# drdh/Homophily-MARL

Measured on AMD Instinct MI355X. Metric: agent_steps_per_sec, higher is better.
Workload: dtype fp32

## Files before the change

homophily_marl_amd/csrc/ssd_policy_mfma.hip:

```cpp
#include "ssd_policy_common.h"
#include <type_traits>

namespace ssd {
#define SSD_GLOBAL __attribute__((address_space(1)))

template <int V> using int_c = std::integral_constant<int, V>;
template <int... Vs, typename R, typename F>
static R pick(int v, R none, F&& f) {
    R r = none;
    ((v == Vs ? (void)(r = f(int_c<Vs>{})) : (void)0), ...);
    return r;
}

static int raise_lds_limit(const void* const* fns, int count, size_t bytes, bool (&done)[64]) {
    int dev = 0;
    if (hipGetDevice(&dev) != hipSuccess || dev < 0 || dev >= 64) return -1;
    if (done[dev]) return 0;
    for (int i = 0; i < count; ++i)
        if (hipFuncSetAttribute(fns[i], hipFuncAttributeMaxDynamicSharedMemorySize, (int)bytes) != hipSuccess) return -1;
    done[dev] = true;
    return 0;
}
static int raise_lds_limit(const void* fn, size_t bytes, bool (&done)[64]) { return raise_lds_limit(&fn, 1, bytes, done); }

// ... 227 lines not shown
    else if (C) asm volatile("s_load_dwordx16 %0, %2, %3\n\ts_load_dwordx4 %1, %2, %4\n\ts_waitcnt lgkmcnt(0)" : "=&s"(a), "=&s"(c) : "s"(ka), "s"(cold_base), "s"(cold_base + 128) : "memory");
    else asm volatile("s_load_dwordx16 %0, %1, %2\n\ts_waitcnt lgkmcnt(0)" : "=&s"(a) : "s"(ka), "s"(cold_base) : "memory");
    A = __builtin_bit_cast(ColdA, a);
    if (B) *B = __builtin_bit_cast(ColdB, b);
    if (C) *C = __builtin_bit_cast(ColdC, c);
#else
    (void)A; (void)B; (void)C;
#endif
}
#define COLD(T, field) cold_ptr<T>(COLD_BASE, (int)offsetof(HeadCold, field))
#define COLD_U64(field) ((uint64_t)cold_ptr<void>(COLD_BASE, (int)offsetof(HeadCold, field)))

template <int PREC>
struct Frag4 { u32x4 h[4], l[4]; };
template <int PREC>
__device__ __forceinline__ void frag4_load(const uint8_t* img, int c, int lane, Frag4<PREC>& f) {
#pragma unroll
    for (int ot = 0; ot < 4; ++ot) {
        const uint8_t* p = img + (size_t)step_piece<PREC>(c, 0, ot) * 1024 + lane * 16;
        f.h[ot] = *reinterpret_cast<const u32x4*>(p);
        if (PREC == 2) f.l[ot] = *reinterpret_cast<const u32x4*>(p + 4 * 1024);
    }
}
template <int PREC>
__device__ __forceinline__ void frag4_mma(const Frag4<PREC>& f, u32x4 bh, u32x4 bl, f32x4* acc) {
    if (PREC == 2) {
#pragma unroll
        for (int ot = 0; ot < 4; ++ot) acc[ot] = mma<PREC>(f.l[ot], bh, acc[ot]);
#pragma unroll
        for (int ot = 0; ot < 4; ++ot) acc[ot] = mma<PREC>(f.h[ot], bl, acc[ot]);
    }
#pragma unroll
    for (int ot = 0; ot < 4; ++ot) acc[ot] = mma<PREC>(f.h[ot], bh, acc[ot]);
}

template <int PREC>
__device__ __forceinline__ void operand(const f32x4 (&x)[4], float scale, u32x4 (&bh)[2], u32x4 (&bl)[2]) {
#pragma unroll
    for (int s = 0; s < 2; ++s) {
        float v[8];
#pragma unroll
        for (int j = 0; j < 8; ++j) v[j] = x[2 * s + (j >> 2)][j & 3] * scale;
        split8<PREC>(v, bh[s], bl[s]);
    }
}

__device__ __forceinline__ float amax2(float acc, float a, float b) {
#if defined(__HIP_DEVICE_COMPILE__)
    float r;
    asm("v_max3_f32 %0, |%1|, |%2|, %3" : "=v"(r) : "v"(a), "v"(b), "v"(acc));
    return r;
#else
    return fmaxf(acc, fmaxf(fabsf(a), fabsf(b)));
#endif
}
template <int NT>
__device__ __forceinline__ float amax_tiles(float acc, const f32x4 (&x)[NT]) {
#pragma unroll
    for (int t = 0; t < NT; ++t) { acc = amax2(acc, x[t][0], x[t][1]); acc = amax2(acc, x[t][2], x[t][3]); }
    return acc;
}

__device__ __forceinline__ float sigmoid_fast(float x) { return __builtin_amdgcn_rcpf(1.f + __expf(-x)); }
__device__ __forceinline__ float tanh_fast(float x) {
    const float ax = fminf(fabsf(x), 15.f);
    const float t = 1.f - 2.f * __builtin_amdgcn_rcpf(__expf(2.f * ax) + 1.f);
    return copysignf(t, x);
}

template <int INC>
struct TileIn {
    f32x4 x[4];
    f32x4 hp[4];
    int pa, act;
    int32_t inc[3];
    uint32_t rv;
    float pr, p0, p1, o0, o1;
    int aj[3];
    float f[3][7];
    float own[3], ep;
    int term;
};

template <typename T>
__device__ __forceinline__ T ld32(const T* base, uint32_t idx) {
    typedef const T SSD_GLOBAL gT;
    return *(gT*)((const uint8_t SSD_GLOBAL*)(const void SSD_GLOBAL*)base + (size_t)(idx * (uint32_t)sizeof(T)));
}
__device__ __forceinline__ void stg128(void* base, size_t byte_off, f32x4 v) {
    typedef f32x4 SSD_GLOBAL gv;
    *(gv*)((uint8_t SSD_GLOBAL*)(void SSD_GLOBAL*)base + byte_off) = v;
}
__device__ __forceinline__ f32x4 ldg128(const void* base, size_t byte_off) {
    typedef const f32x4 SSD_GLOBAL gv;
    return *(gv*)((const uint8_t SSD_GLOBAL*)(const void SSD_GLOBAL*)base + byte_off);
}
template <int INC, bool SMALL = false>
__device__ __forceinline__ void load_tile_rows(const HeadK& a, int tile, int agent, int lane, TileIn<INC>& in) {
    const int m = lane & 15, q = lane >> 4, N = a.N;
    const int b = tile * 16 + m, bc = b < N ? b : N - 1;
    const uint32_t arow = (uint32_t)agent * (uint32_t)N + (uint32_t)bc;
    const uint32_t ro = arow * 64u + 4u * (uint32_t)q;
#pragma unroll
    for (int ct = 0; ct < 4; ++ct) in.hp[ct] = ldg128(a.h, (size_t)((ro + 16u * ct) * 4u));
#pragma unroll
    for (int ct = 0; ct < (INC ? 4 : 2); ++ct) in.x[ct] = ldg128(a.inputs, (size_t)((ro + 16u * ct) * 4u));
    if constexpr (SMALL && !INC) {
        const uint32_t er = (uint32_t)bc * (uint32_t)a.n + (uint32_t)agent;
        in.pa = (int)ld32(reinterpret_cast<const int32_t*>(a.prev_actions), 2u * er);
        in.pr = ld32(a.prev_reward, er);
        in.rv = a.recv ? ld32(reinterpret_cast<const uint32_t*>(a.recv), arow * 4u + (uint32_t)q) : 0u;
        typedef float f32x2v __attribute__((ext_vector_type(2)));
        const f32x2v pp = ld32(reinterpret_cast<const f32x2v*>(a.pos), er);
        in.p0 = pp.x; in.p1 = pp.y;
    }
}
template <int INC, bool ROWS_DONE = false, bool SMALL_DONE = false>
__device__ __forceinline__ void load_tile(const HeadK& a, int tile, int agent, int lane, TileIn<INC>& in) {
    const int m = lane & 15, q = lane >> 4, N = a.N, n = a.n;
    const int b = tile * 16 + m, bc = b < N ? b : N - 1;
    const uint32_t arow = (uint32_t)agent * (uint32_t)N + (uint32_t)bc;
    const uint32_t ro = arow * 64u + 4u * (uint32_t)q;
    if (!ROWS_DONE) {
#pragma unroll
        for (int ct = 0; ct < 4; ++ct) in.hp[ct] = ldg128(a.h, (size_t)((ro + 16u * ct) * 4u));
    }
    if (!INC) {
        if (a.feat_part) {
            const uint32_t rows = (uint32_t)n * (uint32_t)N;
#pragma unroll
            for (int ct = 0; ct < 2; ++ct) {
                f32x4 part[6];
#pragma unroll
                for (int bd = 0; bd < 6; ++bd) {
                    const int bdc = bd < a.feat_bands ? bd : a.feat_bands - 1;
                    part[bd] = ldg128(a.feat_part, (size_t)((((uint32_t)bdc * rows + arow) * 32u + 16u * ct + 4u * q) * 4u));
                }
                f32x4 s = ldg128(a.lin_b, (size_t)((16 * ct + 4 * q) * 4));
#pragma unroll
                for (int bd = 0; bd < 6; ++bd) { const float on = bd < a.feat_bands ? 1.f : 0.f; s += part[bd] * on; }
                in.x[ct] = s;
            }
        } else if (!ROWS_DONE) {
            in.x[0] = ldg128(a.inputs, (size_t)(ro * 4u));
            in.x[1] = ldg128(a.inputs, (size_t)((ro + 16u) * 4u));
        }
        const uint32_t er = (uint32_t)bc * (uint32_t)n + (uint32_t)agent;
        if (!SMALL_DONE) {
            in.pa = (int)ld32(reinterpret_cast<const int32_t*>(a.prev_actions), 2u * er);
            in.pr = ld32(a.prev_reward, er);
        }
        if (a.recv) {
            if (!SMALL_DONE) in.rv = ld32(reinterpret_cast<const uint32_t*>(a.recv), arow * 4u + (uint32_t)q);
            in.inc[0] = in.inc[1] = in.inc[2] = 0;
        } else {
            in.rv = 0u;
            const int32_t* pi = reinterpret_cast<const int32_t*>(a.prev_inc);
#pragma unroll
            for (int k = 0; k < 3; ++k) {
                const int g = q + 4 * k;
                const uint32_t gc = (uint32_t)(g < n ? g : n - 1);
                in.inc[k] = (k == 0 || n > 4 * k) ? ld32(pi, 2u * (((uint32_t)bc * (uint32_t)n + gc) * (uint32_t)n + (uint32_t)agent)) : 0;
            }
        }
        typedef float f32x2v __attribute__((ext_vector_type(2)));
        if (!SMALL_DONE) {
            const f32x2v pp = ld32(reinterpret_cast<const f32x2v*>(a.pos), er);
            in.p0 = pp.x; in.p1 = pp.y;
        }
        const float* orient = a.orient ? a.orient : a.pos;
        const f32x2v oo = ld32(reinterpret_cast<const f32x2v*>(orient), er);
        in.o0 = oo.x; in.o1 = oo.y;
    } else {
        if (!ROWS_DONE) {
#pragma unroll
            for (int ct = 0; ct < 4; ++ct) in.x[ct] = ldg128(a.inputs, (size_t)((ro + 16u * ct) * 4u));
        }
        in.act = (int)ld32(reinterpret_cast<const int32_t*>(a.actions), 2u * ((uint32_t)bc * (uint32_t)n + (uint32_t)agent));
#pragma unroll
        for (int k = 0; k < 3; ++k) {
            const int it = lane + 64 * k, row = it / n, j = it - row * n, bb = tile * 16 + row;
            const bool live = it < 16 * n && bb < N;
            const uint32_t ej = live ? (uint32_t)bb * (uint32_t)n + (uint32_t)j : (uint32_t)N * (uint32_t)n - 1u;
            in.aj[k] = (int)ld32(reinterpret_cast<const int32_t*>(a.actions), 2u * ej);
            typedef float f32x2v __attribute__((ext_vector_type(2)));
            const f32x2v pj = ld32(reinterpret_cast<const f32x2v*>(a.pos_pre), ej), oj = ld32(reinterpret_cast<const f32x2v*>(a.orient_pre), ej);
            in.f[k][0] = pj.x; in.f[k][1] = pj.y; in.f[k][2] = oj.x; in.f[k][3] = oj.y;
            in.f[k][4] = ld32(a.reward, ej); in.f[k][5] = ld32(a.clean, ej); in.f[k][6] = ld32(a.den, ej);
        }
        {
            const int br = tile * 16 + (lane & 15), brc = br < N ? br : N - 1;
            const uint32_t ea = (uint32_t)brc * (uint32_t)n + (uint32_t)agent;
            in.own[0] = ld32(a.reward, ea); in.own[1] = ld32(a.clean, ea); in.own[2] = ld32(a.den, ea);
            in.ep = ld32(a.ep_ret ? a.ep_ret : a.reward, ea);
            in.term = (int)ld32(a.term ? a.term : reinterpret_cast<const uint8_t*>(a.reward), (uint32_t)brc);
        }
    }
}

__device__ __forceinline__ void refetch_head_args(HeadK& out, int k_off) {
#if defined(__HIP_DEVICE_COMPILE__)
    typedef __attribute__((address_space(4))) const uint32_t k_u32;
    uint64_t p = (uint64_t)(uintptr_t)__builtin_amdgcn_kernarg_segment_ptr();
    asm volatile("" : "+s"(p));
    k_u32* src = (k_u32*)(p + (uint64_t)k_off);
    uint32_t* dst = reinterpret_cast<uint32_t*>(&out);
#pragma unroll
    for (int i = 0; i < (int)(sizeof(HeadK) / 4); ++i) dst[i] = src[i];
#else
    (void)out;
#endif
}
static_assert(sizeof(HeadK) % 4 == 0, "HeadK is copied dword by dword");

template <int INC, int PREC, int AT, int GEN, int WAVES, bool LOOP = false, int KOFF = 0, bool PRE_SMALL = false>
__device__ __forceinline__ void head_body(const HeadK& a_entry, uint8_t* lds_raw, const int block) {
    constexpr int COLD_BASE = KOFF + HEAD_COLD_OFFSET;
    constexpr int IMAGE_BYTES = SSD_POLICY_IMAGE_BYTES(PREC);
    constexpr float XS = PREC == 2 ? HEAD_XSCALE : 1.f, INV = PREC == 2 ? 1.f / (HEAD_WSCALE * HEAD_XSCALE) : 1.f;
    const int tid = threadIdx.x, wave = __builtin_amdgcn_readfirstlane(tid >> 6);
    constexpr int A = AT;
    uint32_t seen = 0;
    bool first = true;
    volatile lds_u32* landed = (volatile lds_u32*)(lds_raw + IMAGE_BYTES + WAVES * SCRATCH * 4);
    TileIn<INC> in_rows;
    {
        const HeadK& a = a_entry;
        const int lane = tid & 63;
        (void)lane;
        PSTAMP(0);
        PSTAMP_REAL(14);
        if (!LOOP && wave < WAVES) {
            const int bia0 = block - (block / a.bpa) * a.bpa, tile00 = wave * a.bpa + bia0;
            if (tile00 < ((a.N + 15) >> 4)) load_tile_rows<INC, PRE_SMALL>(a, tile00, block / a.bpa, lane, in_rows);
        }
        if (!LOOP) {
            if (!INC) asm volatile("" :: "s"(a.N), "s"(a.n), "s"(a.bpa), "s"(a.h), "s"(a.inputs), "s"(a.weights), "s"(a.eps), "s"(a.step), "s"(a.t_index),
                                         "s"(a.prev_actions), "s"(a.prev_reward), "s"(a.recv), "s"(a.prev_inc), "s"(a.pos), "s"(a.orient), "s"(a.feat_part),
                                         "s"(a.lin_b), "s"(a.feat_bands), "s"(a.avail_bits), "s"(a.pos_scale));
            else asm volatile("" :: "s"(a.N), "s"(a.n), "s"(a.bpa), "s"(a.h), "s"(a.inputs), "s"(a.weights), "s"(a.eps), "s"(a.step), "s"(a.t_index),
                                    "s"(a.actions), "s"(a.pos_pre), "s"(a.orient_pre), "s"(a.reward), "s"(a.clean), "s"(a.den), "s"(a.ep_ret), "s"(a.term),
                                    "s"(a.inp), "s"(a.pos_scale));
        }
        if (wave == WAVES) *landed = 0u;
        __builtin_amdgcn_s_barrier();
        if (wave == WAVES) {
            const int agent = block / a.bpa;
            stream_image<PREC>(a.weights + (size_t)agent * IMAGE_BYTES + lane * 16, (uint32_t)(uintptr_t)lds_raw, landed);
            return;
        }
    }
    auto pass = [&](const HeadK& a, const int lane, const int tile) {
    const int agent = block / a.bpa;
    const int m = lane & 15, q = lane >> 4;
    const int N = a.N, n = a.n;
    const int tiles = (N + 15) >> 4;
    TileIn<INC> in;
    if constexpr (!LOOP) in = in_rows;
    if (!INC) PSTAMP_DRAINED(8);
    if (!INC) PSTAMP(9);
    float eps = *(const float SSD_GLOBAL*)a.eps;
    int64_t step64 = *(const int64_t SSD_GLOBAL*)a.step;
    long slot_t = a.t_index ? (long)*(const int64_t SSD_GLOBAL*)a.t_index : 0;
    if (tile < tiles) {
        if constexpr (LOOP) load_tile<INC, false>(a, tile, agent, lane, in);
// ... 258 lines not shown
            file_inputs(tile);
            hand_counters();
        }
        if (first) PSTAMP(4);
        u32x4 f2h[2], f2l[2];
#pragma unroll
        for (int s2 = 0; s2 < 2; ++s2) {
            const uint8_t* p2 = img + (size_t)fc2_piece<PREC>(0, s2) * 1024 + lane * 16;
            f2h[s2] = *reinterpret_cast<const u32x4*>(p2);
            if (PREC == 2) f2l[s2] = *reinterpret_cast<const u32x4*>(p2 + 2 * 1024);
        }
        f32x4 hn[4];
#pragma unroll
        for (int ft = 0; ft < 4; ++ft) {
            const f32x4 bir = *reinterpret_cast<const f32x4*>(tail + HT_BI + 16 * ft + 4 * q), bhr = *reinterpret_cast<const f32x4*>(tail + HT_BH + 16 * ft + 4 * q);
            const f32x4 biz = *reinterpret_cast<const f32x4*>(tail + HT_BI + 64 + 16 * ft + 4 * q), bhz = *reinterpret_cast<const f32x4*>(tail + HT_BH + 64 + 16 * ft + 4 * q);
            const f32x4 bin = *reinterpret_cast<const f32x4*>(tail + HT_BI + 128 + 16 * ft + 4 * q), bhn = *reinterpret_cast<const f32x4*>(tail + HT_BH + 128 + 16 * ft + 4 * q);
#pragma unroll
            for (int r = 0; r < 4; ++r) {
                const float rg = sigmoid_fast(fmaf(g[ft][r], INV, bir[r] + bhr[r]));
                const float zg = sigmoid_fast(fmaf(g[4 + ft][r], INV, biz[r] + bhz[r]));
                const float ng = tanh_fast(fmaf(g[8 + ft][r], INV, bin[r]) + rg * fmaf(g[12 + ft][r], INV, bhn[r]));
                hn[ft][r] = (1.f - zg) * ng + zg * hp[ft][r];
            }
            if (valid) stg128(h_row, (size_t)((16 * ft + 4 * q) * 4), hn[ft]);
        }
        if (first) PSTAMP(5);
        f32x4 o2 = f32x4{0.f, 0.f, 0.f, 0.f};
        operand<PREC>(hn, XS, bh, bl);
#pragma unroll
        for (int s2 = 0; s2 < 2; ++s2) {
            if (PREC == 2) { o2 = mma<PREC>(f2l[s2], bh[s2], o2); o2 = mma<PREC>(f2h[s2], bl[s2], o2); }
            o2 = mma<PREC>(f2h[s2], bh[s2], o2);
        }
        {
            const f32x4 b2 = *reinterpret_cast<const f32x4*>(tail + HT_B2 + 4 * q);
#pragma unroll
            for (int r = 0; r < 4; ++r) o2[r] = fmaf(o2[r], INV, b2[r]);
        }
        *reinterpret_cast<f32x4*>(scratch + m * 16 + 4 * q) = o2;
        __builtin_amdgcn_fence(__ATOMIC_ACQ_REL, "wavefront");
        __builtin_amdgcn_wave_barrier();
        if (!INC) {
            const int bb = tile * 16 + lane;
            ColdA ca;
            cold_blocks(COLD_BASE, ca, nullptr, nullptr);
            auto out_actions = ca.out_actions; auto p_act = ca.p_act; auto d_actions = ca.d_actions;
            auto out_i32 = ca.out_actions_i32;
            auto q_out = ca.q_out; auto d_onehot = ca.d_onehot;
            if (lane < 16 && bb < N) {
                float av[16];
#pragma unroll
                for (int k4 = 0; k4 < 4; ++k4) {
                    const f32x4 t4 = *reinterpret_cast<const f32x4*>(scratch + lane * 16 + 4 * k4);
                    av[4 * k4] = t4[0]; av[4 * k4 + 1] = t4[1]; av[4 * k4 + 2] = t4[2]; av[4 * k4 + 3] = t4[3];
                }
                const float val = av[A];
                const uint32_t rq = (uint32_t)(agent * N + bb);
                const uint32_t rk = (a.env_id_base + (uint32_t)bb) * (uint32_t)n + (uint32_t)agent;
                const int act = dueling_pick_bits<AT>(av, val, A, avail_bits, eps, step, a.seed, rk, q_out ? q_out + (size_t)rq * A : (decltype(q_out))nullptr);
                out_actions[(size_t)bb * n + agent] = act;
                if (out_i32) out_i32[(size_t)bb * n + agent] = act;
                if (p_act) p_act[(size_t)bb * n + agent] = act;
                if constexpr (GEN >= 2) {
                    auto rec_out = cold_ptr<uint8_t>(COLD_BASE, gather_slots<0>() + 16);
                    if (rec_out) rec_out[(size_t)bb * 16 + agent] = (uint8_t)act;
                }
                if (d_actions && file) {
                    const size_t sr = ((size_t)bb * a.slots + slot_t) * n + agent;
                    d_actions[sr] = act;
#pragma unroll
                    for (int k = 0; k < A; ++k) d_onehot[sr * A + k] = k == act ? 1.f : 0.f;
                }
            }
        } else {
            if (first) PSTAMP(8);
            const float* w2o = tail + HT_W2O;
            ColdA ca; ColdB cb;
            cold_blocks(COLD_BASE, ca, &cb, nullptr);
            auto out_actions = ca.out_actions; auto p_inc = cb.p_inc; auto d_actions_inc = cb.d_actions_inc;
            auto q_out = ca.q_out;
            auto recv_out = COLD(uint8_t, recv_out);
            if (first) PSTAMP(9);
            const uint32_t n_magic = (65536u + (uint32_t)n - 1u) / (uint32_t)n;
#pragma unroll
            for (int k = 0; k < 3; ++k) {
                if (first && k == 1) PSTAMP(10);
                if (first && k == 2) PSTAMP(11);
                const int it = lane + 64 * k;
                const int row = (int)(((uint32_t)it * n_magic) >> 16), j = it - row * n, bb = tile * 16 + row;
                if (it >= 16 * n || bb >= N) continue;
                const int aj = in.aj[k];
                float f[7];
                f[0] = in.f[k][0] / a.pos_scale; f[1] = in.f[k][1] / a.pos_scale;
#pragma unroll
                for (int e = 2; e < 7; ++e) f[e] = in.f[k][e];
                const f32x4 sc = *reinterpret_cast<const f32x4*>(scratch + row * 16);
                const f32x4 wa = *reinterpret_cast<const f32x4*>(w2o + aj * 4);
                float av[4];
#pragma unroll
                for (int o = 0; o < 4; ++o) av[o] = sc[o] + wa[o];
#pragma unroll
                for (int e = 0; e < 7; ++e) {
                    const f32x4 we = *reinterpret_cast<const f32x4*>(w2o + (A + e) * 4);
#pragma unroll
                    for (int o = 0; o < 4; ++o) av[o] = fmaf(f[e], we[o], av[o]);
                }
                const uint32_t rq = (uint32_t)((agent * N + bb) * n + j);
                const uint32_t rk = ((a.env_id_base + (uint32_t)bb) * (uint32_t)n + (uint32_t)agent) * (uint32_t)n + (uint32_t)j;
                int act = dueling_pick_bits<3>(av, av[3], 3, 0xFFFFFFFFu, eps, step, a.seed, rk, q_out ? q_out + (size_t)rq * 3 : (decltype(q_out))nullptr);
                if (j == agent) act = 0;
                const size_t pair = ((size_t)bb * n + agent) * n + j;
                out_actions[pair] = act;
                if (p_inc) p_inc[pair] = act;
                if (recv_out) recv_out[((size_t)j * N + bb) * 16 + agent] = (uint8_t)act;
                if (d_actions_inc && file) d_actions_inc[(((size_t)bb * a.slots + slot_t) * n + agent) * n + j] = act;
            }
            const int br = tile * 16 + lane;
            if (lane < 16 && br < N && cb.d_reward) {
                const size_t ea = (size_t)br * n + agent, sr = ((size_t)br * a.slots + slot_t) * n + agent;
                if (file) { cb.d_reward[sr] = in.own[0]; cb.d_clean[sr] = in.own[1]; cb.d_den[sr] = in.own[2]; }
                if (cb.p_rew) cb.p_rew[ea] = in.own[0];
                if (cb.ep_ret) cb.ep_ret[ea] = in.ep + in.own[0];
                if (agent == 0 && cb.d_term && file) cb.d_term[(size_t)br * a.slots + slot_t] = (uint8_t)in.term;
            }
        }
        __builtin_amdgcn_wave_barrier();
        if (first) PSTAMP(6);
        first = false;
#undef SSD_LOAD_STEP
    };
    if (tile < tiles) run_tile();
    else hand_counters();
    };
    const int lane0 = tid & 63;
    {
        const int bia = block - (block / a_entry.bpa) * a_entry.bpa;
        const int tile0 = wave * a_entry.bpa + bia;
        if constexpr (!LOOP) {
            pass(a_entry, lane0, tile0);
        } else {
            const int stride = a_entry.bpa * WAVES, tiles_all = (a_entry.N + 15) >> 4;
            int tile = tile0;
            do {
                HeadK al;
                refetch_head_args(al, KOFF);
                int lane = lane0;
#if defined(__HIP_DEVICE_COMPILE__)
                asm volatile("" : "+v"(lane));
#endif
                pass(al, lane, tile);
                tile += stride;
#if defined(__HIP_DEVICE_COMPILE__)
                asm volatile("" : "+s"(tile));
#endif
            } while (tile < tiles_all);
        }
    }
    {
        const HeadK& a = a_entry;
        const int lane = lane0;
        (void)a; (void)lane;
        PSTAMP(7);
        PSTAMP_REAL(15);
    }
}

constexpr int HEAD_WAVES = 8;
constexpr int HEAD_WAVES_LOOP = 8;
constexpr int HEAD_WAVES_GATHER = 7;
constexpr int head_waves(bool loop, int gen = 0) { return gen >= 2 ? HEAD_WAVES_GATHER : loop ? HEAD_WAVES_LOOP : HEAD_WAVES; }
constexpr int HEAD_LEAD_BYTES = 2 * 4 + 6 * 8;
template <int INC, int PREC, int AT, int GEN = 0, bool LOOP = false>
__global__ __launch_bounds__((head_waves(LOOP, GEN) + 1) * 64) void k_head(uint32_t p_Nn, int p_bpa, float* p_h, float* p_inputs, const int64_t* p_prev_actions,
                                                                      const float* p_prev_reward, const uint8_t* p_recv, const float* p_pos, HeadK a, HeadCold cold_unused) {
    extern __shared__ __attribute__((aligned(16))) uint8_t lds_raw[];
    if constexpr (LOOP) head_body<INC, PREC, AT, GEN, head_waves(LOOP, GEN), LOOP, HEAD_LEAD_BYTES>(a, lds_raw, (int)blockIdx.x);
    else {
        HeadK al = a;
        al.N = (int)(p_Nn & 0xFFFFFFu); al.n = (int)(p_Nn >> 24); al.bpa = p_bpa; al.h = p_h; al.inputs = p_inputs;
        if constexpr (!INC) { al.prev_actions = p_prev_actions; al.prev_reward = p_prev_reward; al.recv = p_recv; al.pos = p_pos; }
        head_body<INC, PREC, AT, GEN, head_waves(LOOP, GEN), LOOP, HEAD_LEAD_BYTES, !INC>(al, lds_raw, (int)blockIdx.x);
    }
}

static bool head_gathers(const ssd_policy_head* p) { return p->input_flags && (p->input_flags & SSD_INPUT_OTHERS_LAST_ACTION); }
static bool head_gathers_onehot(const ssd_policy_head* p) { return p->input_flags && (p->input_flags & SSD_INPUT_GATHER_ONEHOT); }
static int chip_cus() {
    static int cus[64] = {};
    int dev = 0;
    if (hipGetDevice(&dev) != hipSuccess || dev < 0 || dev >= 64) return 256;
    if (!cus[dev]) {
        int v = 0;
        cus[dev] = (hipDeviceGetAttribute(&v, hipDeviceAttributeMultiprocessorCount, dev) == hipSuccess && v > 0) ? v : 256;
    }
    return cus[dev];
}
static void head_args(const ssd_policy_head* p, HeadK& k, HeadCold& c) {
    k.N = p->n_env; k.n = p->n_agents; k.A = p->n_actions; k.inp = p->input_shape;
    k.pos_scale = p->pos_scale; k.seed = p->seed; k.env_id_base = p->env_id_base;
    k.inputs = p->inputs; k.h = p->h; k.weights = static_cast<const uint8_t*>(p->weights); k.avail = p->avail; k.eps = p->epsilon; k.step = p->step;
    k.prev_actions = p->prev_actions; k.prev_reward = p->prev_reward; k.prev_inc = p->prev_actions_inc; k.pos = p->pos; k.orient = p->orient;
    k.actions = p->actions; k.pos_pre = p->pos_pre; k.orient_pre = p->orient_pre; k.reward = p->reward; k.clean = p->clean_num;
    k.den = p->apple_den;
    k.t_index = p->t_index; k.slots = p->t_index ? p->t_slots : 1;
    k.feat_part = p->feat_part; k.feat_bands = p->feat_bands; k.lin_b = p->lin_b;
    k.ep_ret = p->ep_return; k.term = p->terminated;
// ... 151 lines not shown
        } else {
            const int s = F - HF_FC2, k = 32 * s + 16 * (j >> 2) + 4 * q + (j & 3);
            if (m < p.fc2_out) w = p.fc2_w[((size_t)agent * p.fc2_in + k) * p.fc2_out + m];
            else if (m == p.fc2_out) w = p.fc2_v_w[(size_t)agent * p.fc2_in + k];
            piece = fc2_piece<PREC>(0, s); term_pieces = 2;
        }
        store_term<PREC>(img + ((size_t)piece * 64 + lane) * 16 + 2 * j, w * WS, (size_t)term_pieces * 1024, err);
    }
    if (e < HT_TOT) {
        float v = 0.f;
        if (e < HT_BI) v = p.fc1_b[(size_t)agent * 64 + e];
        else if (e < HT_BH) { const int i = e - HT_BI; v = p.b_i[i >> 6][(size_t)agent * 64 + (i & 63)]; }
        else if (e < HT_B2) { const int i = e - HT_BH; v = p.b_h[i >> 6][(size_t)agent * 64 + (i & 63)]; }
        else if (e < HT_W2O) {
            const int o = e - HT_B2;
            if (o < p.fc2_out) v = p.fc2_b[(size_t)agent * p.fc2_out + o]; else if (o == p.fc2_out) v = p.fc2_v_b[agent];
        } else {
            const int i = e - HT_W2O, ee = i >> 2, o = i & 3;
            if (64 + ee < p.fc2_in) {
                if (o < p.fc2_out) v = p.fc2_w[((size_t)agent * p.fc2_in + 64 + ee) * p.fc2_out + o];
                else if (o == p.fc2_out) v = p.fc2_v_w[(size_t)agent * p.fc2_in + 64 + ee];
            }
        }
        reinterpret_cast<float*>(img + (size_t)tail_piece<PREC>() * 1024)[e] = v;
    }
}
template <int PREC>
__global__ __launch_bounds__(256) void k_pack_head(ssd_policy_head_params p, uint8_t* image, int32_t* err) { pack_head_body<PREC, 0>(p, image, err); }
template <int PREC>
__global__ __launch_bounds__(256) void k_pack_head_others(ssd_policy_head_params p, uint8_t* image, int32_t* err) { pack_head_body<PREC, 1>(p, image, err); }
template <int PREC>
__global__ __launch_bounds__(256) void k_pack_head_onehot(ssd_policy_head_params p, uint8_t* image, int32_t* err) { pack_head_body<PREC, 2>(p, image, err); }

void launch_pack_head(const ssd_policy_head_params* p, int prec, void* image, hipStream_t s) {
    const dim3 grid((HF_TOT * 512 + 255) / 256, p->n_agents);
    int32_t* err = numeric_err_word();
    const int mode = (p->input_flags & SSD_INPUT_GATHER_ONEHOT) ? 2 : (p->input_flags & SSD_INPUT_OTHERS_LAST_ACTION) ? 1 : 0;
    pick<2, 1>(prec == 2 ? 2 : 1, 0, [&](auto pr) {
        constexpr int PREC = decltype(pr)::value;
        if (mode == 2) hipLaunchKernelGGL(k_pack_head_onehot<PREC>, grid, dim3(256), 0, s, *p, static_cast<uint8_t*>(image), err);
        else if (mode == 1) hipLaunchKernelGGL(k_pack_head_others<PREC>, grid, dim3(256), 0, s, *p, static_cast<uint8_t*>(image), err);
        else hipLaunchKernelGGL(k_pack_head<PREC>, grid, dim3(256), 0, s, *p, static_cast<uint8_t*>(image), err);
        return 0;
    });
}

template <int V> struct Geo;
template <> struct Geo<15> { static constexpr int O = 13, CP = 16, NXT = 2, XTP = 1, R = 13, NB = 1; };
template <> struct Geo<31> { static constexpr int O = 29, CP = 32, NXT = 4, XTP = 2, R = 10, NB = 3; };
static_assert(Geo<15>::R == SSD_ENCODE_BAND_ROWS(15) && Geo<15>::NB == SSD_ENCODE_BANDS(15) && Geo<31>::R == SSD_ENCODE_BAND_ROWS(31) &&
              Geo<31>::NB == SSD_ENCODE_BANDS(31), "the shipped bands are the header's geometry");
constexpr int ENC_BT_MAX = 5;
constexpr int ENC_WAVES = 8;
template <int V> constexpr int enc_row_bytes() { return 3 * Geo<V>::CP + 8 * Geo<V>::NXT; }
template <int V> constexpr int enc_batch_row_bytes() {
    int b = (Geo<V>::R + 2) * enc_row_bytes<V>();
    while ((b & 255) % 16 != 8) b += 8;
    return b;
}
template <int V, int PREC, int BT = ENC_BT_MAX> constexpr size_t enc_lds_bytes() {
    const size_t work = (size_t)BT * 16 * enc_batch_row_bytes<V>() + (size_t)PREC * 9 * 1024;
    const size_t red = (size_t)ENC_WAVES * BT * 2 * 1024;
    return work > red ? work : red;
}

struct EncK {
    const uint8_t* codes; long code_bytes, env_stride, slot_stride, agent_stride; const int64_t* slot_t;
    int slot_add;
    int rows, n, agent_major;
    const uint8_t *conv_frags, *lin_frags;
    const float *conv_b, *lin_b;
    float* out; int out_stride;
    float* part;
    float* act;
    int64_t* slot_t_copy; int64_t* counter_inc;
    int mask_alphabet;
    int layout;
    PSTAMP_DECL
};

template <int BT>
__device__ __forceinline__ void enc_reduce_finish(const EncK& a, uint8_t* lds_raw, const f32x4 (&accl)[BT][2], int row0, int band, float INV, int tid, int lane,
                                                  int wave) {
    __syncthreads();
    f32x4* red = reinterpret_cast<f32x4*>(lds_raw);
#pragma unroll
    for (int bt = 0; bt < BT; ++bt)
#pragma unroll
        for (int mt = 0; mt < 2; ++mt) red[((wave * BT + bt) * 2 + mt) * 64 + lane] = accl[bt][mt];
    __syncthreads();
    for (int it = tid; it < BT * 2 * 64; it += ENC_WAVES * 64) {
        const int l = it & 63, mt = (it >> 6) & 1, bt = it >> 7;
        f32x4 sum = red[((0 * BT + bt) * 2 + mt) * 64 + l];
#pragma unroll
        for (int w = 1; w < ENC_WAVES; ++w) sum += red[((w * BT + bt) * 2 + mt) * 64 + l];
        const int row = row0 + bt * 16 + (l & 15), f0 = 16 * mt + 4 * (l >> 4);
        if (row < a.rows) {
            const int b = row / a.n, i = row - b * a.n;
            const size_t orow = a.agent_major ? (size_t)i * (a.rows / a.n) + b : (size_t)row;
            if (a.part) {
                f32x4 o;
#pragma unroll
                for (int r = 0; r < 4; ++r) o[r] = sum[r] * INV;
                *reinterpret_cast<f32x4*>(a.part + ((size_t)band * a.rows + orow) * 32 + f0) = o;
            } else {
#pragma unroll
                for (int r = 0; r < 4; ++r) a.out[orow * a.out_stride + f0 + r] = leaky(fmaf(sum[r], INV, a.lin_b[f0 + r]));
            }
        }
    }
}

template <int V, int PREC, bool ACT, int BT>
__device__ __forceinline__ void encode_body(const EncK& a, uint8_t* lds_raw, const int block_x, const int block_y) {
    using G = Geo<V>;
    constexpr int O = G::O, CP = G::CP, XTP = G::XTP, R = G::R;
    constexpr int RB = enc_row_bytes<V>(), PR = enc_batch_row_bytes<V>();
    constexpr int PLANES = BT * 16 * PR, CONV_BYTES = PREC * 9 * 1024;
    constexpr uint32_t ON = PREC == 2 ? 0x3Cu : 0x3Fu;
    constexpr float CS = PREC == 2 ? ENC_CSCALE : 1.f, INV = PREC == 2 ? 1.f / (ENC_CSCALE * ENC_LSCALE) : 1.f;
    uint8_t* planes = lds_raw;
    uint8_t* cfr = lds_raw + PLANES;
    const int tid = threadIdx.x, lane = tid & 63, wave = __builtin_amdgcn_readfirstlane(tid >> 6);
    const int m = lane & 15, q = lane >> 4;
    const int row0 = block_x * (BT * 16);
    const int band = block_y, y0 = band * R;
    const int Rb = O - y0 < R ? O - y0 : R;
    const long t_off = a.slot_t ? ((long)(*a.slot_t) + a.slot_add) * a.slot_stride : 0;
    PSTAMP(0);
    PSTAMP_REAL(14);
    if (block_x == 0 && block_y == 0 && tid == 0) {
        if (a.slot_t_copy) *a.slot_t_copy = *a.slot_t;
        if (a.counter_inc) *a.counter_inc += 1;
    }
    {
        const u32x4* src = reinterpret_cast<const u32x4*>(a.conv_frags);
        u32x4* dst = reinterpret_cast<u32x4*>(cfr);
        constexpr int NV = CONV_BYTES / 16, PER = (NV + ENC_WAVES * 64 - 1) / (ENC_WAVES * 64);
        u32x4 tmp[PER];
#pragma unroll
        for (int j = 0; j < PER; ++j) { const int e = tid + j * ENC_WAVES * 64; if (e < NV) tmp[j] = src[e]; }
        constexpr int NQ = CP / 16, ITEMS = BT * 16 * (R + 2), NT = ENC_WAVES * 64, IPT = (ITEMS + NT - 1) / NT;
        typedef uint32_t u32x4_u __attribute__((ext_vector_type(4), aligned(1)));
        typedef __attribute__((address_space(1))) u32x4_u gl_u32x4_u;
        typedef __attribute__((address_space(1))) uint32_t gl_u32;
        u32x4 cw[IPT][NQ];
        const uintptr_t cbase = reinterpret_cast<uintptr_t>(a.codes), cend = cbase + (uintptr_t)a.code_bytes;
#pragma unroll
        for (int k = 0; k < IPT; ++k) {
            const int it = tid + k * NT;
            const int yy = it % (R + 2), r = it / (R + 2);
            const int row = row0 + r, y = y0 + yy;
#pragma unroll
            for (int h = 0; h < NQ; ++h) cw[k][h] = u32x4{0u, 0u, 0u, 0u};
            if (it < ITEMS && row < a.rows && y < V) {
                const int b = row / a.n, i = row - b * a.n;
                const uintptr_t ptr = cbase + (uintptr_t)((long)b * a.env_stride + t_off + (long)i * a.agent_stride + y * V);
                if (ptr + 16 * NQ <= cend) {
#pragma unroll
                    for (int h = 0; h < NQ; ++h) cw[k][h] = *reinterpret_cast<const gl_u32x4_u*>(ptr + 16 * h);
                } else {
                    const uintptr_t al = ptr & ~(uintptr_t)3, lim = (cend + 3) & ~(uintptr_t)3;
                    uint32_t prev = *reinterpret_cast<const gl_u32*>(al);
#pragma unroll
                    for (int h = 0; h < NQ; ++h)
#pragma unroll
                        for (int e = 0; e < 4; ++e) {
                            const uintptr_t nx = al + 4 * (4 * h + e + 1);
                            const uint32_t next = nx + 4 <= lim ? *reinterpret_cast<const gl_u32*>(nx) : 0u;
                            cw[k][h][e] = __builtin_amdgcn_alignbyte(next, prev, (uint32_t)(ptr & 3));
                            prev = next;
                        }
                }
            }
        }
#pragma unroll
        for (int k = 0; k < IPT; ++k) {
            const int it = tid + k * NT;
            if (it >= ITEMS) continue;
            const int yy = it % (R + 2), r = it / (R + 2);
            uint8_t* d = planes + (size_t)r * PR + yy * RB;
            u32x4 pl[3][NQ];
#pragma unroll
            for (int h = 0; h < NQ; ++h) {
                u32x4 c = cw[k][h];
                if (h == NQ - 1) c[3] &= 0x00FFFFFFu;
#pragma unroll
                for (int e = 0; e < 4; ++e) {
                    const uint32_t b0 = c[e] & 0x01010101u, b1 = (c[e] >> 1) & 0x01010101u;
                    if (a.mask_alphabet) {
                        pl[0][h][e] = b0 * ON; pl[1][h][e] = b1 * ON; pl[2][h][e] = ((c[e] >> 2) & 0x01010101u) * ON;
// ... 828 lines not shown
```

Before: 335.2 million.

## Skip self-pairs in inclusion head and restructure encoder reduce epilogue

The per-pair inclusion head now iterates over 16*(n-1) non-self pairs instead of 16*n, mapping indices past the agent's own slot. The self pair's action is written as zero separately, and its Q values are computed only when q_out is requested. The encoder reduction epilogue precomputes output offsets and bias before the barrier, assigns items to waves statically, and emits vectorized 128-bit global stores. This cuts wasted loads and arithmetic and shortens the tail after the barrier, at the cost of extra code paths and a static assumption of 8 encoder waves.

```diff
diff --git a/homophily_marl_amd/csrc/ssd_policy_mfma.hip b/homophily_marl_amd/csrc/ssd_policy_mfma.hip
--- a/homophily_marl_amd/csrc/ssd_policy_mfma.hip
+++ b/homophily_marl_amd/csrc/ssd_policy_mfma.hip
@@ -333,6 +333,18 @@
     int term;
 };
 
+struct IncItems {
+    int n1, count;
+    uint32_t magic;
+    __device__ __forceinline__ explicit IncItems(int n) : n1(n - 1), count(16 * (n - 1)), magic((65536u + (uint32_t)(n > 1 ? n - 1 : 1) - 1u) / (uint32_t)(n > 1 ? n - 1 : 1)) {}
+    __device__ __forceinline__ bool pass(int k) const { return count > 64 * k; }
+    __device__ __forceinline__ void pair(int it, int agent, int& row, int& j) const {
+        row = (int)(((uint32_t)it * magic) >> 16);
+        const int jj = it - row * n1;
+        j = jj + (jj >= agent ? 1 : 0);
+    }
+};
+
 template <typename T>
 __device__ __forceinline__ T ld32(const T* base, uint32_t idx) {
     typedef const T SSD_GLOBAL gT;
@@ -428,10 +440,15 @@
             for (int ct = 0; ct < 4; ++ct) in.x[ct] = ldg128(a.inputs, (size_t)((ro + 16u * ct) * 4u));
         }
         in.act = (int)ld32(reinterpret_cast<const int32_t*>(a.actions), 2u * ((uint32_t)bc * (uint32_t)n + (uint32_t)agent));
+        const IncItems items(n);
 #pragma unroll
         for (int k = 0; k < 3; ++k) {
-            const int it = lane + 64 * k, row = it / n, j = it - row * n, bb = tile * 16 + row;
-            const bool live = it < 16 * n && bb < N;
+            if (!items.pass(k)) break;
+            int row, j;
+            const int it = lane + 64 * k;
+            items.pair(it, agent, row, j);
+            const int bb = tile * 16 + row;
+            const bool live = it < items.count && bb < N;
             const uint32_t ej = live ? (uint32_t)bb * (uint32_t)n + (uint32_t)j : (uint32_t)N * (uint32_t)n - 1u;
             in.aj[k] = (int)ld32(reinterpret_cast<const int32_t*>(a.actions), 2u * ej);
             typedef float f32x2v __attribute__((ext_vector_type(2)));
@@ -856,34 +873,42 @@
             auto q_out = ca.q_out;
             auto recv_out = COLD(uint8_t, recv_out);
             if (first) PSTAMP(9);
-            const uint32_t n_magic = (65536u + (uint32_t)n - 1u) / (uint32_t)n;
+            auto pair_q = [&](int row, int aj, const float (&fj)[7], float (&av)[4]) {
+                float f[7];
+                f[0] = fj[0] / a.pos_scale; f[1] = fj[1] / a.pos_scale;
+#pragma unroll
+                for (int e = 2; e < 7; ++e) f[e] = fj[e];
+                const f32x4 sc = *reinterpret_cast<const f32x4*>(scratch + row * 16);
+                const f32x4 wa = *reinterpret_cast<const f32x4*>(w2o + aj * 4);
+#pragma unroll
+                for (int o = 0; o < 4; ++o) av[o] = sc[o] + wa[o];
+#pragma unroll
+                for (int e = 0; e < 7; ++e) {
+                    const f32x4 we = *reinterpret_cast<const f32x4*>(w2o + (A + e) * 4);
+#pragma unroll
+                    for (int o = 0; o < 4; ++o) av[o] = fmaf(f[e], we[o], av[o]);
+                }
+            };
+            const IncItems items(n);
+            int lane_items = lane;
+#if defined(__HIP_DEVICE_COMPILE__)
+            asm volatile("" : "+v"(lane_items));
+#endif
 #pragma unroll
             for (int k = 0; k < 3; ++k) {
+                if (!items.pass(k)) break;
                 if (first && k == 1) PSTAMP(10);
                 if (first && k == 2) PSTAMP(11);
-                const int it = lane + 64 * k;
-                const int row = (int)(((uint32_t)it * n_magic) >> 16), j = it - row * n, bb = tile * 16 + row;
-                if (it >= 16 * n || bb >= N) continue;
-                const int aj = in.aj[k];
-                float f[7];
-                f[0] = in.f[k][0] / a.pos_scale; f[1] = in.f[k][1] / a.pos_scale;
-#pragma unroll
-                for (int e = 2; e < 7; ++e) f[e] = in.f[k][e];
-                const f32x4 sc = *reinterpret_cast<const f32x4*>(scratch + row * 16);
-                const f32x4 wa = *reinterpret_cast<const f32x4*>(w2o + aj * 4);
+                const int it = lane_items + 64 * k;
+                int row, j;
+                items.pair(it, agent, row, j);
+                const int bb = tile * 16 + row;
+                if (it >= items.count || bb >= N) continue;
                 float av[4];
-#pragma unroll
-                for (int o = 0; o < 4; ++o) av[o] = sc[o] + wa[o];
-#pragma unroll
-                for (int e = 0; e < 7; ++e) {
-                    const f32x4 we = *reinterpret_cast<const f32x4*>(w2o + (A + e) * 4);
-#pragma unroll
-                    for (int o = 0; o < 4; ++o) av[o] = fmaf(f[e], we[o], av[o]);
-                }
+                pair_q(row, in.aj[k], in.f[k], av);
                 const uint32_t rq = (uint32_t)((agent * N + bb) * n + j);
                 const uint32_t rk = ((a.env_id_base + (uint32_t)bb) * (uint32_t)n + (uint32_t)agent) * (uint32_t)n + (uint32_t)j;
-                int act = dueling_pick_bits<3>(av, av[3], 3, 0xFFFFFFFFu, eps, step, a.seed, rk, q_out ? q_out + (size_t)rq * 3 : (decltype(q_out))nullptr);
-                if (j == agent) act = 0;
+                const int act = dueling_pick_bits<3>(av, av[3], 3, 0xFFFFFFFFu, eps, step, a.seed, rk, q_out ? q_out + (size_t)rq * 3 : (decltype(q_out))nullptr);
                 const size_t pair = ((size_t)bb * n + agent) * n + j;
                 out_actions[pair] = act;
                 if (p_inc) p_inc[pair] = act;
@@ -891,12 +916,43 @@
                 if (d_actions_inc && file) d_actions_inc[(((size_t)bb * a.slots + slot_t) * n + agent) * n + j] = act;
             }
             const int br = tile * 16 + lane;
+            if (lane < 16 && br < N) {
+                const size_t self = ((size_t)br * n + agent) * n + agent;
+                out_actions[self] = 0;
+                if (p_inc) p_inc[self] = 0;
+                if (recv_out) recv_out[((size_t)agent * N + br) * 16 + agent] = (uint8_t)0;
+                if (d_actions_inc && file) d_actions_inc[(((size_t)br * a.slots + slot_t) * n + agent) * n + agent] = 0;
+            }
             if (lane < 16 && br < N && cb.d_reward) {
                 const size_t ea = (size_t)br * n + agent, sr = ((size_t)br * a.slots + slot_t) * n + agent;
                 if (file) { cb.d_reward[sr] = in.own[0]; cb.d_clean[sr] = in.own[1]; cb.d_den[sr] = in.own[2]; }
                 if (cb.p_rew) cb.p_rew[ea] = in.own[0];
                 if (cb.ep_ret) cb.ep_ret[ea] = in.ep + in.own[0];
                 if (agent == 0 && cb.d_term && file) cb.d_term[(size_t)br * a.slots + slot_t] = (uint8_t)in.term;
+            }
+            if (q_out) {
+                int lane_q = lane;
+#if defined(__HIP_DEVICE_COMPILE__)
+                asm volatile("" : "+v"(lane_q));
+#endif
+                const int br_q = tile * 16 + lane_q;
+                if (lane_q < 16 && br_q < N) {
+                    const uint32_t ea = (uint32_t)br_q * (uint32_t)n + (uint32_t)agent;
+                    typedef float f32x2v __attribute__((ext_vector_type(2)));
+                    auto acts = cold_ptr<const int32_t>(KOFF, (int)offsetof(HeadK, actions));
+                    auto pos_pre = cold_ptr<const f32x2v>(KOFF, (int)offsetof(HeadK, pos_pre));
+                    auto orient_pre = cold_ptr<const f32x2v>(KOFF, (int)offsetof(HeadK, orient_pre));
+                    auto rew = cold_ptr<const float>(KOFF, (int)offsetof(HeadK, reward));
+                    auto cln = cold_ptr<const float>(KOFF, (int)offsetof(HeadK, clean));
+                    auto den = cold_ptr<const float>(KOFF, (int)offsetof(HeadK, den));
+                    const int a_self = (int)acts[2u * ea];
+                    const f32x2v pj = pos_pre[ea], oj = orient_pre[ea];
+                    const float fs[7] = {pj.x, pj.y, oj.x, oj.y, rew[ea], cln[ea], den[ea]};
+                    float av[4];
+                    pair_q(lane_q, a_self, fs, av);
+                    const uint32_t rq = (uint32_t)((agent * N + br_q) * n + agent);
+                    (void)dueling_pick_bits<3>(av, av[3], 3, 0xFFFFFFFFu, 0.f, step, a.seed, 0u, q_out + (size_t)rq * 3);
+                }
             }
         }
         __builtin_amdgcn_wave_barrier();
@@ -1214,31 +1270,47 @@
 template <int BT>
 __device__ __forceinline__ void enc_reduce_finish(const EncK& a, uint8_t* lds_raw, const f32x4 (&accl)[BT][2], int row0, int band, float INV, int tid, int lane,
                                                   int wave) {
+    constexpr int NU = (BT * 2 * 64 + ENC_WAVES * 64 - 1) / (ENC_WAVES * 64);
+    static_assert(ENC_WAVES == 8, "an item's (lane, mt, bt) from (lane, wave)");
+    typedef float f32x4_u __attribute__((ext_vector_type(4), aligned(4)));
+    const int mt = wave & 1, f0 = 16 * mt + 4 * (lane >> 4);
+    const bool to_part = a.part != nullptr;
+    f32x4 bias = {0.f, 0.f, 0.f, 0.f};
+    if (!to_part) bias = *reinterpret_cast<const f32x4_u SSD_GLOBAL*>((const float SSD_GLOBAL*)a.lin_b + f0);
+    size_t off[NU];
+    bool on[NU];
+#pragma unroll
+    for (int u = 0; u < NU; ++u) {
+        const int bt = (wave >> 1) + 4 * u, row = row0 + bt * 16 + (lane & 15);
+        on[u] = bt < BT && row < a.rows;
+        const int b = row / a.n, i = row - b * a.n;
+        const size_t orow = a.agent_major ? (size_t)i * (a.rows / a.n) + b : (size_t)row;
+        off[u] = to_part ? ((size_t)band * a.rows + orow) * 32 + f0 : orow * a.out_stride + f0;
+    }
     __syncthreads();
     f32x4* red = reinterpret_cast<f32x4*>(lds_raw);
 #pragma unroll
     for (int bt = 0; bt < BT; ++bt)
 #pragma unroll
-        for (int mt = 0; mt < 2; ++mt) red[((wave * BT + bt) * 2 + mt) * 64 + lane] = accl[bt][mt];
+        for (int mt2 = 0; mt2 < 2; ++mt2) red[((wave * BT + bt) * 2 + mt2) * 64 + lane] = accl[bt][mt2];
     __syncthreads();
-    for (int it = tid; it < BT * 2 * 64; it += ENC_WAVES * 64) {
-        const int l = it & 63, mt = (it >> 6) & 1, bt = it >> 7;
-        f32x4 sum = red[((0 * BT + bt) * 2 + mt) * 64 + l];
-#pragma unroll
-        for (int w = 1; w < ENC_WAVES; ++w) sum += red[((w * BT + bt) * 2 + mt) * 64 + l];
-        const int row = row0 + bt * 16 + (l & 15), f0 = 16 * mt + 4 * (l >> 4);
-        if (row < a.rows) {
-            const int b = row / a.n, i = row - b * a.n;
-            const size_t orow = a.agent_major ? (size_t)i * (a.rows / a.n) + b : (size_t)row;
-            if (a.part) {
-                f32x4 o;
-#pragma unroll
-                for (int r = 0; r < 4; ++r) o[r] = sum[r] * INV;
-                *reinterpret_cast<f32x4*>(a.part + ((size_t)band * a.rows + orow) * 32 + f0) = o;
-            } else {
-#pragma unroll
-                for (int r = 0; r < 4; ++r) a.out[orow * a.out_stride + f0 + r] = leaky(fmaf(sum[r], INV, a.lin_b[f0 + r]));
-            }
+#pragma unroll
+    for (int u = 0; u < NU; ++u) {
+        const int bt = (wave >> 1) + 4 * u;
+        if (u > 0 && bt >= BT) break;
+        f32x4 sum = red[((0 * BT + bt) * 2 + mt) * 64 + lane];
+#pragma unroll
+        for (int w = 1; w < ENC_WAVES; ++w) sum += red[((w * BT + bt) * 2 + mt) * 64 + lane];
+        if (!on[u]) continue;
+        f32x4 o;
+        if (to_part) {
+#pragma unroll
+            for (int r = 0; r < 4; ++r) o[r] = sum[r] * INV;
+            *reinterpret_cast<f32x4 SSD_GLOBAL*>((float SSD_GLOBAL*)a.part + off[u]) = o;
+        } else {
+#pragma unroll
+            for (int r = 0; r < 4; ++r) o[r] = leaky(fmaf(sum[r], INV, bias[r]));
+            *reinterpret_cast<f32x4_u SSD_GLOBAL*>((float SSD_GLOBAL*)a.out + off[u]) = o;
         }
     }
 }
```

After: 343.6 million (median of 6 runs). +2.5%, better.
